# PaddlePaddle/PaddleRobotics

Measured on NVIDIA H100. Metric: env-steps/sec (A1, 4096 envs), higher is better.
Workload: dtype f32

## Files before the change

paddlerobotics_b200/csrc/b2q_api.cu:

```cuda
#include <cuda_runtime.h>
#include <cstdio>
#include <cstdlib>
#include <new>
#include <string>
#include "b2q_host_common.h"
#include "b2q_render_internal.h"
#include "../../include/b2q_render.h"

using namespace b2q;

namespace {

struct WarpComm {
  int k;
  unsigned char* scr;
  __device__ __forceinline__ int leg() const { return k; }
  template <typename T> __device__ __forceinline__ T* scratch() const { return reinterpret_cast<T*>(scr); }
  __device__ __forceinline__ void sync() const { __syncwarp(); }
  __device__ __forceinline__ bool any(bool f) const { return __any_sync(0xffffffffu, f) != 0; }
  template <typename T>
  __device__ __forceinline__ T sum4(T v) const {
    v += __shfl_xor_sync(0xffffffffu, v, 1);
    v += __shfl_xor_sync(0xffffffffu, v, 2);
    return v;
  }
  template <typename T>
  __device__ __forceinline__ T bcast(T v, int f) const { return __shfl_sync(0xffffffffu, v, f, 4); }
};

template <typename T>
__device__ __forceinline__ const Model<T>& stage_model(const Model<T>* g, unsigned char* smem) {
  Model<T>* s = reinterpret_cast<Model<T>*>(smem);
  const uint4* src = reinterpret_cast<const uint4*>(g);
  uint4* dst = reinterpret_cast<uint4*>(s);
  constexpr int NV = (int)((sizeof(Model<T>) + 15) / 16);
  for (int i0 = threadIdx.x; i0 < NV; i0 += 4 * blockDim.x) {
    uint4 v[4];
#pragma unroll
    for (int k = 0; k < 4; k++) { const int i = i0 + k * (int)blockDim.x; if (i < NV) v[k] = __ldg(src + i); }
#pragma unroll
    for (int k = 0; k < 4; k++) { const int i = i0 + k * (int)blockDim.x; if (i < NV) dst[i] = v[k]; }
  }
  __syncthreads();
  return *s;
}

template <typename T>
__device__ __forceinline__ void copy_block(T* __restrict__ dst, const T* stage, int n) {
  constexpr int PER = 16 / (int)sizeof(T);
  if ((((size_t)dst | (size_t)stage) & 15) == 0 && n % PER == 0) {
    uint4* d4 = reinterpret_cast<uint4*>(dst); const uint4* s4 = reinterpret_cast<const uint4*>(stage);
    for (int i = threadIdx.x; i < n / PER; i += blockDim.x) d4[i] = s4[i];
  } else {
    for (int i = threadIdx.x; i < n; i += blockDim.x) dst[i] = stage[i];
  }
}

template <typename T>
__device__ __forceinline__ void emit_obs_block(const Model<T>& md, const T* stage, T* __restrict__ obs, int env0, int rows) {
  const int od = md.obs_dim;
  T* dst = obs + (size_t)env0 * od;
  if (md.obs_identity) { copy_block(dst, stage, rows * OBS_DIM); return; }
  for (int i = threadIdx.x; i < rows * od; i += blockDim.x) { int r = i / od, j = i - r * od; dst[i] = obs_out_elem(md, stage + r * OBS_DIM, j); }
}

template <typename T, int FEAT>
__global__ void __launch_bounds__(128) b2q_step_kernel(Cfg<T> cf, const Model<T>* __restrict__ gm, Buffers<T> B, const T* __restrict__ action, int donef,
                                                       int auto_reset, T* __restrict__ obs, T* __restrict__ reward, uint8_t* __restrict__ done, T* __restrict__ info) {
  extern __shared__ __align__(32) unsigned char smem[];
  const Model<T>& md = stage_model(gm, smem);
  T* stage = reinterpret_cast<T*>(smem + ((sizeof(Model<T>) + 31) & ~size_t(31)));
  int gid = blockIdx.x * blockDim.x + threadIdx.x;
  int env = gid >> 2;
  const int env0 = (blockIdx.x * blockDim.x) >> 2, per_cta = blockDim.x >> 2;
  bool valid = env < B.N;
  const int srow = env0 + (int)(threadIdx.x >> 2);
  if (!valid) env = B.N - 1;
  T* istage0 = stage + (size_t)per_cta * OBS_DIM;
  WarpComm cm{(int)(threadIdx.x & 3), reinterpret_cast<unsigned char*>(istage0 + (size_t)per_cta * INFO_DIM + (size_t)(threadIdx.x >> 2) * scratch_floats(FEAT))};
  T* istage = istage0;
  step_lane<T, FEAT>(cm, cf, md, B, env, valid, action, donef, auto_reset, stage + (ptrdiff_t)(srow - env) * OBS_DIM, reward, done, istage, env0, env0);
  __syncthreads();
  const int rows = min(per_cta, B.N - env0);
  emit_obs_block(md, stage, obs, env0, rows);
  copy_block(info + (size_t)env0 * INFO_DIM, istage, rows * INFO_DIM);
}

template <typename T, int FEAT>
__global__ void __launch_bounds__(128) b2q_settle_kernel(Cfg<T> cf, const Model<T>* __restrict__ gm, Buffers<T> B, const uint8_t* __restrict__ mask) {
  extern __shared__ __align__(32) unsigned char smem[];
  const Model<T>& md = stage_model(gm, smem);
  int gid = blockIdx.x * blockDim.x + threadIdx.x;
  int env = gid >> 2;
  bool valid = env < B.N;
  if (!valid) env = B.N - 1;
  if (mask && !mask[env]) valid = false;
  T* scr0 = reinterpret_cast<T*>(smem + ((sizeof(Model<T>) + 31) & ~size_t(31))) + (size_t)(blockDim.x >> 2) * (OBS_DIM + INFO_DIM);
  WarpComm cm{(int)(threadIdx.x & 3), reinterpret_cast<unsigned char*>(scr0 + (size_t)(threadIdx.x >> 2) * scratch_floats(FEAT))};
  settle_lane<T, FEAT>(cm, cf, md, B, env, valid);
}

template <typename T>
__global__ void __launch_bounds__(128) b2q_reset_kernel(Cfg<T> cf, const Model<T>* __restrict__ gm, Buffers<T> B, const uint8_t* __restrict__ mask, const T* __restrict__ xoff,
                                                        T* __restrict__ obs) {
  extern __shared__ __align__(32) unsigned char smem[];
  const Model<T>& md = stage_model(gm, smem);
  T* stage = reinterpret_cast<T*>(smem + ((sizeof(Model<T>) + 31) & ~size_t(31)));
  int gid = blockIdx.x * blockDim.x + threadIdx.x;
  int env = gid >> 2;
  const int env0 = (blockIdx.x * blockDim.x) >> 2;
  bool valid = env < B.N;
  if (!valid) env = B.N - 1;
  if (mask && !mask[env]) valid = false;
  WarpComm cm{(int)(threadIdx.x & 3), nullptr};
  T* srow = stage + (size_t)(threadIdx.x >> 2) * OBS_DIM;
  reset_lane<T>(cm, cf, md, B, env, valid, obs ? srow : (T*)nullptr, xoff);
  if (obs) {
    __syncwarp();
    if (valid) { const int od = md.obs_dim; for (int j = threadIdx.x & 3; j < od; j += 4) obs[(size_t)env * od + j] = obs_out_elem(md, srow, j); }
  }
  (void)env0;
}

template <typename T>
__global__ void b2q_pack_param_kernel(const T* __restrict__ dyn, const T* __restrict__ def48, P4<T>* param, const uint8_t* __restrict__ mask, int N, T max_latency,
                                      int* __restrict__ overflow) {
  int env = blockIdx.x * blockDim.x + threadIdx.x;
  if (env >= N || (mask && !mask[env])) return;
  pack_param_env<T>(dyn, def48, param, N, env);
  const T lat = dyn ? dyn[(size_t)env * 48 + 25] : def48[25];
  if (!(lat <= max_latency)) atomicMax(overflow, 1);
}
template <typename T>
__global__ void b2q_pack_force_kernel(const T* __restrict__ f, P4<T>* extf, int N) {
// ... 46 lines not shown
  do {                                                                                \
    cudaError_t e_ = (call);                                                          \
    if (e_ != cudaSuccess) {                                                          \
      err = std::string(#call) + ": " + cudaGetErrorString(e_);                       \
      return B2Q_ECUDA;                                                               \
    }                                                                                 \
  } while (0)

template <typename T>
struct EnvT : EnvBase {
  Cfg<T> kc;
  Buffers<T> B;
  Model<T>* d_model = nullptr;
  T* d_def48 = nullptr;
  T* d_hf = nullptr;
  void* d_pool = nullptr;
  int tpb = 32;
  float hf_lo = 0.0f, hf_hi = 0.0f;

  ~EnvT() override {
    cudaSetDevice(cfg.device);
    if (d_pool) cudaFree(d_pool);
    if (d_model) cudaFree(d_model);
    if (d_def48) cudaFree(d_def48);
    if (d_hf) cudaFree(d_hf);
    if (st_act) cudaFree(st_act);
    if (h_flag) cudaFreeHost(h_flag);
  }
  int grid_lanes() const { return (B.N * 4 + tpb - 1) / tpb; }

  int init(const B2QConfig& c) {
    cfg = c; prec = c.precision;
    tpb = c.threads_per_block ? c.threads_per_block : 32;
    if (const char* e = std::getenv("B2Q_HOST_IO")) host_io = std::atoi(e);
    CK(cudaSetDevice(c.device));
    int N = c.num_envs, Dm = c.ring_depth;
    if (c.terrain_type == 1) {
      size_t n = (size_t)c.hf_nx * c.hf_ny;
      T* tmp = (T*)malloc(n * sizeof(T));
      if (!tmp) { err = "host alloc failed"; return B2Q_ENOMEM; }
      for (size_t i = 0; i < n; i++) tmp[i] = (T)c.hf_host[i];
      hf_lo = hf_hi = (float)tmp[0];
      for (size_t i = 0; i < n; i++) { hf_lo = std::fmin(hf_lo, (float)tmp[i]); hf_hi = std::fmax(hf_hi, (float)tmp[i]); }
      cudaError_t e1 = cudaMalloc(&d_hf, n * sizeof(T));
      if (e1 == cudaSuccess) e1 = cudaMemcpy(d_hf, tmp, n * sizeof(T), cudaMemcpyHostToDevice);
      free(tmp);
      CK(e1);
    }
    kc = make_cfg<T>(c, d_hf);
    Model<T> hm; build_model_host(hm, c.foot_radius, c.etg_T, c.etg_amp, c.etg_phase0, c.etg_phase1, c.etg_foot_y_inset);
    build_obs_map(hm, c); obs_dim = hm.obs_dim;
    feat = config_feat(c);
    if (feat) tpb = 32;
    if (smem_bytes() > 48 * 1024) {
      if (feat) {
        CK(cudaFuncSetAttribute(b2q_step_kernel<T, 1>, cudaFuncAttributeMaxDynamicSharedMemorySize, (int)smem_bytes()));
        CK(cudaFuncSetAttribute(b2q_settle_kernel<T, 1>, cudaFuncAttributeMaxDynamicSharedMemorySize, (int)smem_bytes()));
      } else {
        CK(cudaFuncSetAttribute(b2q_step_kernel<T, 0>, cudaFuncAttributeMaxDynamicSharedMemorySize, (int)smem_bytes()));
        CK(cudaFuncSetAttribute(b2q_settle_kernel<T, 0>, cudaFuncAttributeMaxDynamicSharedMemorySize, (int)smem_bytes()));
      }
    }
    CK(cudaHostAlloc((void**)&h_flag, sizeof(int), cudaHostAllocDefault));
    CK(cudaMalloc((void**)&d_model, (sizeof(Model<T>) + 15) / 16 * 16));
    CK(cudaMemset(d_model, 0, (sizeof(Model<T>) + 15) / 16 * 16));
    CK(cudaMemcpy(d_model, &hm, sizeof(Model<T>), cudaMemcpyHostToDevice));
    double d48[48]; default_dyn_row(d48); T t48[48]; for (int i = 0; i < 48; i++) t48[i] = (T)d48[i];
    CK(cudaMalloc(&d_def48, sizeof(t48)));
    CK(cudaMemcpy(d_def48, t48, sizeof(t48), cudaMemcpyHostToDevice));
    size_t packs = (size_t)(NS + NS + 12 + NP + NE + Dm * 24 + STUCK_H + 1) * N;
    size_t bytes = packs * sizeof(P4<T>) + (size_t)(N + 1) * sizeof(int);
    CK(cudaMalloc(&d_pool, bytes));
    CK(cudaMemset(d_pool, 0, bytes));
    P4<T>* p = (P4<T>*)d_pool;
    B.N = N; B.Dm = Dm;
    B.state = p; p += (size_t)NS * N; B.snap = p; p += (size_t)NS * N; B.snap_obs = p; p += (size_t)12 * N;
    B.param = p; p += (size_t)NP * N; B.etg = p; p += (size_t)NE * N; B.ring = p; p += (size_t)Dm * 24 * N;
    B.pos_hist = p; p += (size_t)STUCK_H * N; B.extf = p; p += (size_t)N;
    B.step_count = (int*)p; d_flag = B.step_count + N;
    int rc = set_dynamics(nullptr, nullptr, 0);
    if (rc) return rc;
    rc = reset(nullptr, nullptr, nullptr, nullptr, nullptr, 0);
    if (rc) return rc;
    CK(cudaDeviceSynchronize());
    return B2Q_OK;
  }
  size_t smem_bytes() const {
    return ((sizeof(Model<T>) + 31) & ~size_t(31)) + (size_t)(tpb / 4) * (OBS_DIM + INFO_DIM + scratch_floats(feat)) * sizeof(T);
  }

  int set_dynamics(const uint8_t* mask, const void* dyn, cudaStream_t s) override {
    CK(cudaSetDevice(cfg.device));
    int N = B.N;
    const double max_lat = ((double)B.Dm * cfg.action_repeat - 2) * cfg.sim_dt * (1.0 + 1e-9);
    CK(cudaMemsetAsync(d_flag, 0, sizeof(int), s));
    b2q_pack_param_kernel<T><<<(N + 127) / 128, 128, 0, s>>>((const T*)dyn, d_def48, const_cast<P4<T>*>(B.param), mask, N, (T)max_lat, d_flag);
    CK(cudaMemcpyAsync(h_flag, d_flag, sizeof(int), cudaMemcpyDeviceToHost, s));
    CK(cudaStreamSynchronize(s));
    launches += 1;
    if (*h_flag) {
      char buf[200];
      snprintf(buf, sizeof buf, "b2q_set_dynamics: a control_latency exceeds %.4f s, the most ring_depth=%d can serve (need ring_depth >= ceil((latency/sim_dt + 2) / action_repeat))", max_lat, B.Dm);
      err = buf;
      return B2Q_EINVAL;
    }
    if (feat) b2q_settle_kernel<T, 1><<<grid_lanes(), tpb, smem_bytes(), s>>>(kc, d_model, B, mask);
    else b2q_settle_kernel<T, 0><<<grid_lanes(), tpb, smem_bytes(), s>>>(kc, d_model, B, mask);
    launches += 1;
    CK(cudaGetLastError());
    return B2Q_OK;
  }
  int reset(const uint8_t* mask, const void* w, const void* b, const void* xoff, void* obs, cudaStream_t s) override {
    CK(cudaSetDevice(cfg.device));
    int N = B.N;
    if (w || b) { b2q_pack_etg_kernel<T><<<(N + 127) / 128, 128, 0, s>>>((const T*)w, (const T*)b, const_cast<P4<T>*>(B.etg), mask, N); launches++; }
    const size_t smem_reset = ((sizeof(Model<T>) + 31) & ~size_t(31)) + (size_t)(tpb / 4) * OBS_DIM * sizeof(T);
    b2q_reset_kernel<T><<<grid_lanes(), tpb, smem_reset, s>>>(kc, d_model, B, mask, (const T*)xoff, (T*)obs);
    launches++;
    CK(cudaGetLastError());
    return B2Q_OK;
  }
  int set_force(const void* f, cudaStream_t s) override {
    if (!cfg.external_force) { err = "b2q_set_external_force: the handle was created with external_force = 0"; return B2Q_EINVAL; }
    CK(cudaSetDevice(cfg.device));
    b2q_pack_force_kernel<T><<<(B.N + 127) / 128, 128, 0, s>>>((const T*)f, const_cast<P4<T>*>(B.extf), B.N);
    launches++;
    CK(cudaGetLastError());
    return B2Q_OK;
  }
  int feat = 0; int* d_flag = nullptr; int* h_flag = nullptr;
  int step(const void* action, int donef, void* obs, void* rew, uint8_t* done, void* info, cudaStream_t s) override {
    if (!action || !obs || !rew || !done || !info) { err = "b2q_step: null device pointer"; return B2Q_EINVAL; }
    { int cur = -1; if (cudaGetDevice(&cur) != cudaSuccess || cur != cfg.device) CK(cudaSetDevice(cfg.device)); }
    if (feat) b2q_step_kernel<T, 1><<<grid_lanes(), tpb, smem_bytes(), s>>>(kc, d_model, B, (const T*)action, donef, cfg.auto_reset, (T*)obs, (T*)rew, done, (T*)info);
    else b2q_step_kernel<T, 0><<<grid_lanes(), tpb, smem_bytes(), s>>>(kc, d_model, B, (const T*)action, donef, cfg.auto_reset, (T*)obs, (T*)rew, done, (T*)info);
    launches++;
    CK(cudaGetLastError());
    return B2Q_OK;
  }
  T* st_act = nullptr; T* st_obs = nullptr; T* st_rew = nullptr; uint8_t* st_done = nullptr; T* st_info = nullptr;
  int step_host(const void* a, int donef, void* obs, void* rew, uint8_t* done, void* info, cudaStream_t s) override {
    if (!a || !obs || !rew || !done) { err = "b2q_step_host: null host pointer"; return B2Q_EINVAL; }
    CK(cudaSetDevice(cfg.device));
    const size_t N = (size_t)B.N;
    if (!st_act) {
      size_t bytes = N * ((size_t)act_dim() + OBS_DIM + 1 + INFO_DIM) * sizeof(T) + N + 512;
      void* p = nullptr;
      CK(cudaMalloc(&p, bytes));
      st_act = (T*)p; st_obs = st_act + N * (size_t)act_dim(); st_rew = st_obs + N * OBS_DIM; st_done = (uint8_t*)(st_rew + N);
      st_info = (T*)((uint8_t*)p + ((N * ((size_t)act_dim() + OBS_DIM + 1) * sizeof(T) + N + 255) / 256) * 256);
    }
    const T* act_dev = st_act;
    if (host_io >= 1 && (act_dev = (const T*)mapped(a)) == nullptr) act_dev = st_act;
    if (act_dev == st_act) CK(cudaMemcpyAsync(st_act, a, N * (size_t)act_dim() * sizeof(T), cudaMemcpyHostToDevice, s));
    T* obs_dev = nullptr; T* rew_dev = nullptr; uint8_t* done_dev = nullptr;
    if (host_io >= 2) { obs_dev = (T*)mapped(obs); rew_dev = (T*)mapped(rew); done_dev = (uint8_t*)mapped(done); }
    const bool direct = obs_dev && rew_dev && done_dev;
    T* info_dev = (direct && info) ? (T*)mapped(info) : nullptr;
    int rc = direct ? step(act_dev, donef, obs_dev, rew_dev, done_dev, info_dev ? info_dev : st_info, s) : step(act_dev, donef, st_obs, st_rew, st_done, st_info, s);
    if (rc) return rc;
    if (info_dev) info = nullptr;
    const size_t b_obs = N * (size_t)obs_dim * sizeof(T), b_rew = N * sizeof(T);
    if (direct) {
    } else if ((uint8_t*)rew == (uint8_t*)obs + b_obs && done == (uint8_t*)rew + b_rew) {
      CK(cudaMemcpyAsync(obs, st_obs, b_obs + b_rew + N, cudaMemcpyDeviceToHost, s));
    } else {
      CK(cudaMemcpyAsync(obs, st_obs, b_obs, cudaMemcpyDeviceToHost, s));
      CK(cudaMemcpyAsync(rew, st_rew, b_rew, cudaMemcpyDeviceToHost, s));
      CK(cudaMemcpyAsync(done, st_done, N, cudaMemcpyDeviceToHost, s));
    }
    if (info) CK(cudaMemcpyAsync(info, st_info, N * INFO_DIM * sizeof(T), cudaMemcpyDeviceToHost, s));
    CK(cudaStreamSynchronize(s));
    return B2Q_OK;
  }
  int host_io = 2;
  void* mapped(const void* p) {
    cudaPointerAttributes at;
    if (cudaPointerGetAttributes(&at, p) == cudaSuccess && at.type == cudaMemoryTypeHost && at.devicePointer) return at.devicePointer;
    cudaGetLastError();
    return nullptr;
  }
  int get_state(void* out, cudaStream_t s) override {
    if (!out) { err = "b2q_get_state: null pointer"; return B2Q_EINVAL; }
    CK(cudaSetDevice(cfg.device));
    b2q_get_state_kernel<T><<<(B.N + 127) / 128, 128, 0, s>>>(B.state, (T*)out, B.N); launches++;
    CK(cudaGetLastError());
    return B2Q_OK;
// ... 98 lines not shown
```

paddlerobotics_b200/csrc/b2q_sim.cuh:

```cuda
#pragma once
#include "b2q_math.cuh"

namespace b2q {

constexpr int NS = 37;
constexpr int NP = 15;
constexpr int NE = 16;
constexpr int OBS_DIM = 49;
constexpr int INFO_DIM = 56;
constexpr int ETG_H = 20;

template <typename T>
struct alignas(4 * sizeof(T)) P4 {
  T x, y, z, w;
};

template <typename T>
struct LegModel {
  T p1[3];
  T lhip;
  T com[3][3];
  T I[3][6];
  T m[3];
};
template <typename T>
struct Model {
  LegModel<T> leg[4];
  T m0, I0[6];
  T foot_r, l_up, l_low;
  T etg_u[ETG_H][2];
  T base_foot[4][3];
  T etg_mean[12], etg_std[12], etg_istd[12];
  T pose_ori[3];
  T qlo[3], qhi[3];
  T knee_r;
  int obs_dim, obs_identity;
  int obs_src[OBS_DIM];
  T obs_scale[OBS_DIM], obs_shift[OBS_DIM];
};
template <typename T>
struct Cfg {
  T dt; int R; int iters; T erp, warm, margin; int interp; T tau_limit; int settle_steps;
  int filter; T fb0, fb1, fb2, fa1, fa2; int etg; int max_steps;
  T etg_T, etg_T2, etg_sigma_sq, etg_amp, etg_ph0, etg_ph1;
  T w_torso, w_feet, w_up, w_tau, w_stand, w_badfoot, w_footcontact, w_done, reward_p, vel_d;
  int terrain, hf_nx, hf_ny; T hf_x0, hf_y0, hf_cell, hf_icell, idt; const T* hf;
  int clip_cmd; T max_dq;
  int noise_on; T noise[5]; unsigned long long noise_seed;
  int stuck, body_coll;
  int motor_mode, jlim, extf, knee; T damp[4];
};
constexpr int STUCK_H = 10;
template <typename T>
struct Buffers {
  int N, Dm;
  P4<T>* state;
  P4<T>* snap;
  P4<T>* snap_obs;
  const P4<T>* param;
  const P4<T>* etg;
  P4<T>* ring;
  int* step_count;
  P4<T>* pos_hist;
  const P4<T>* extf;
};
template <typename T>
struct LaneParam {
// ... 44 lines not shown
  K.a2 = K.R1.cy;
  K.p1 = mk<T>(lm.p1[0], lm.p1[1], lm.p1[2]);
  K.p2 = K.p1 + K.R1.cy * lm.lhip;
  K.p3 = K.p2 - K.R2.cz * md.l_up;
  K.toe = K.p3 - K.R3m.cz * md.l_low;
}

template <typename T>
B2Q_HD void leg_ik(const Model<T>& md, V3<T> f, T lhip, T* ang) {
  T lu = md.l_up, ll = md.l_low;
  T tk = -m_acos((f.x * f.x + f.y * f.y + f.z * f.z - lhip * lhip - ll * ll - lu * lu) / (2 * ll * lu));
  T l = m_sqrt(lu * lu + ll * ll + 2 * lu * ll * m_cos(tk));
  T th = m_asin(-f.x / l) - tk / 2;
  T cc = m_cos(th + tk / 2);
  T c1 = lhip * f.y - l * cc * f.z;
  T s1 = l * cc * f.y + lhip * f.z;
  ang[0] = m_atan2(s1, c1); ang[1] = th; ang[2] = tk;
}

template <typename T, class Comm>
B2Q_HD void etg_act_leg(const Comm& cm, const Cfg<T>& cf, const Model<T>& md, const P4<T>* etg, int N, int env, T t, T* act) {
  const int k = cm.leg();
  if (!cf.etg) { act[0] = act[1] = act[2] = T(0); return; }
  const T two_pi = T(6.283185307179586476925286766559);
  T tt = (k == 0 || k == 3) ? t : t + T(0.5) * cf.etg_T2;
  T om = two_pi / cf.etg_T;
  T x0 = cf.etg_amp * m_sin(cf.etg_ph0 + om * tt), x1 = cf.etg_amp * m_sin(cf.etg_ph1 + om * tt);
  T d[3] = {0, 0, 0};
  const T isig = T(1) / cf.etg_sigma_sq;
  T e[4 * NE];
#pragma unroll
  for (int p = 0; p < NE; p++) { P4<T> v = ldp(etg, p, N, env); e[4 * p] = v.x; e[4 * p + 1] = v.y; e[4 * p + 2] = v.z; e[4 * p + 3] = v.w; }
#pragma unroll
  for (int h = 0; h < ETG_H; h++) {
    T dx = x0 - md.etg_u[h][0], dy = x1 - md.etg_u[h][1];
    T r = m_exp(-(dx * dx + dy * dy) * isig);
#pragma unroll
    for (int a = 0; a < 3; a++) d[a] += e[a * ETG_H + h] * r;
  }
#pragma unroll
  for (int a = 0; a < 3; a++) d[a] += e[60 + a];
  const LegModel<T>& lm = md.leg[k];
  T ang[3];
  for (int tries = 0; tries < 200; tries++) {
    V3<T> f = mk<T>(md.base_foot[k][0] + d[0] - lm.p1[0], md.base_foot[k][1] + d[1] - lm.p1[1], md.base_foot[k][2] + d[2] - lm.p1[2]);
    leg_ik(md, f, lm.lhip, ang);
    if (!(m_isnan(ang[0]) || m_isnan(ang[1]) || m_isnan(ang[2]))) break;
    d[0] *= T(0.95); d[1] *= T(0.95); d[2] *= T(0.95);
  }
#pragma unroll
  for (int a = 0; a < 3; a++) act[a] = ang[a] - md.pose_ori[a];
}

constexpr int RPL = 9, NRW = 4 * RPL;
constexpr int SCRATCH_FLOATS = NRW * 6 + 4 * 45 + NRW * 4 + NRW * NRW;
constexpr int SCRATCH_FAST = 272;
B2Q_HD constexpr int scratch_floats(int feat) { return feat ? SCRATCH_FLOATS : SCRATCH_FAST; }
#define JLIM_GAP T(0.06)
template <typename T, class Comm>
B2Q_HD void solve_rows36(const Comm& cm, const Cfg<T>& cf, T mu, const T (*Y)[6] , const T* u , const T* blk45 ,
                         const T* targ , const bool* act , const T* warm , T* lk ) {
  const int k = cm.leg();
  T* sh = cm.template scratch<T>();
  T* Ya = sh; T* blk = sh + NRW * 6; T* vec = blk + 4 * 45; T* W = vec + NRW * 4;
  cm.sync();
  for (int e = 0; e < RPL; e++) {
    const int r = RPL * k + e;
    for (int c = 0; c < 6; c++) Ya[r * 6 + c] = Y[e][c];
    vec[r * 4 + 0] = u[e]; vec[r * 4 + 1] = targ[e]; vec[r * 4 + 2] = act[e] ? T(1) : T(0); vec[r * 4 + 3] = warm[e];
  }
  for (int i = 0; i < 45; i++) blk[k * 45 + i] = blk45[i];
  cm.sync();
  const int grp_row[9] = {6, 7, 8, 0, 3, 1, 2, 4, 5}, grp_par[9] = {-1, -1, -1, -1, -1, 0, 0, 3, 3};
  int idx[NRW], par[NRW], pos_of[NRW], n = 0;
  for (int i = 0; i < NRW; i++) pos_of[i] = -1;
  for (int seg = 0; seg < 5; seg++) {
    const int g0 = seg == 0 ? 0 : seg == 1 ? 3 : seg == 2 ? 4 : seg == 3 ? 5 : 7, g1 = seg == 0 ? 3 : seg == 1 ? 4 : seg == 2 ? 5 : seg == 3 ? 7 : 9;
    for (int f = 0; f < 4; f++)
      for (int g = g0; g < g1; g++) {
        const int r = RPL * f + grp_row[g];
        if (!(vec[r * 4 + 2] > T(0))) continue;
        idx[n] = r; par[n] = grp_par[g] >= 0 ? pos_of[RPL * f + grp_par[g]] : -1; pos_of[r] = n; n++;
      }
  }
  for (int i = 0; i < n; i++) {
    const int r = idx[i];
    if (r / RPL != k) continue;
    for (int j = 0; j < n; j++) {
      const int c = idx[j];
      T acc = T(0);
      for (int q = 0; q < 6; q++) acc += Ya[r * 6 + q] * Ya[c * 6 + q];
      if (c / RPL == k) { const int a = r - RPL * k, b = c - RPL * k; acc += blk[k * 45 + (a >= b ? a * (a + 1) / 2 + b : b * (b + 1) / 2 + a)]; }
      W[i * NRW + j] = acc;
    }
  }
  cm.sync();
  T lam[NRW], uu[NRW];
  for (int i = 0; i < n; i++) lam[i] = vec[idx[i] * 4 + 3];
  for (int i = 0; i < n; i++) { T a = vec[idx[i] * 4 + 0]; for (int j = 0; j < n; j++) a += W[i * NRW + j] * lam[j]; uu[i] = a; }
  for (int it = 0; it < cf.iters; it++) {
    for (int i = 0; i < n; i++) {
      T ln = lam[i] + (vec[idx[i] * 4 + 1] - uu[i]) / W[i * NRW + i];
      if (par[i] >= 0) { T lim = mu * lam[par[i]]; ln = m_min(m_max(ln, -lim), lim); } else ln = m_max(ln, T(0));
      T dl = ln - lam[i]; lam[i] = ln;
      for (int j = 0; j < n; j++) uu[j] += W[j * NRW + i] * dl;
    }
  }
  for (int e = 0; e < RPL; e++) { const int q = pos_of[RPL * k + e]; lk[e] = q >= 0 ? lam[q] : T(0); }
  cm.sync();
}

template <typename T, int FEAT, class Comm>
B2Q_HD void substep(const Comm& cm, const Cfg<T>& cf, const Model<T>& md, const LaneParam<T>& pr, LaneState<T>& s,
                    const T* target, T* tau_out, V3<T> fext = V3<T>{0, 0, 0}, const T* hyb = nullptr ) {
  const int k = cm.leg();
  const LegModel<T>& lm = md.leg[k];
  const T dt = cf.dt, idt = cf.idt;
  R3<T> R = quat_to_R(s.qx, s.qy, s.qz, s.qw);
  V3<T> wB = rotT(R, s.vang), vB = rotT(R, s.vlin), gB = rotT(R, pr.g);

  T tau[3];
#pragma unroll
  for (int j = 0; j < 3; j++) {
    T cmd = target[j];
    if (cf.clip_cmd) cmd = m_min(m_max(cmd, s.q[j] - cf.max_dq), s.q[j] + cf.max_dq);
    T t = T(-1) * (pr.kp[j] * (s.q[j] - cmd)) - pr.kd[j] * (s.qd[j] - T(0));
    if (FEAT && cf.motor_mode == 1) t = target[j];
    if (FEAT && cf.motor_mode == 2) t = T(-1) * (hyb[j] * (s.q[j] - cmd)) - hyb[6 + j] * (s.qd[j] - hyb[3 + j]) + hyb[9 + j];
    if (cf.tau_limit > T(0)) t = m_min(m_max(t, -cf.tau_limit), cf.tau_limit);
    tau[j] = t; tau_out[j] = t;
  }

  LegKin<T> K; leg_kin(md, lm, s.q, K);
  const V3<T> a1 = mk<T>(1, 0, 0), a2 = K.a2;
  V3<T> cL[3]; S3<T> IL[3]; T mL[3];
  {
    const R3<T>* Rs[3] = {&K.R1, &K.R2, &K.R3m};
    const V3<T> ps[3] = {K.p1, K.p2, K.p3};
#pragma unroll
    for (int i = 0; i < 3; i++) {
      cL[i] = ps[i] + rot(*Rs[i], mk<T>(lm.com[i][0], lm.com[i][1], lm.com[i][2]));
      S3<T> Il = {lm.I[i][0], lm.I[i][1], lm.I[i][2], lm.I[i][3], lm.I[i][4], lm.I[i][5]};
      S3<T> Ib = rot_sym(*Rs[i], Il);
      T sc = pr.iscale[i];
      IL[i].xx = Ib.xx * sc; IL[i].xy = Ib.xy * sc; IL[i].xz = Ib.xz * sc; IL[i].yy = Ib.yy * sc; IL[i].yz = Ib.yz * sc; IL[i].zz = Ib.zz * sc;
      mL[i] = lm.m[i] * pr.mscale[i];
    }
  }
  V3<T> w1 = wB + a1 * s.qd[0], w2 = w1 + a2 * s.qd[1], w3 = w2 + a2 * s.qd[2];
  V3<T> pdd0 = cross(wB, vB) - gB;
  V3<T> al1 = cross(wB, a1) * s.qd[0];
  V3<T> pdd1 = pdd0 + cross(wB, cross(wB, K.p1));
  V3<T> al2 = al1 + cross(w1, a2) * s.qd[1];
  V3<T> d21 = K.p2 - K.p1;
  V3<T> pdd2 = pdd1 + cross(al1, d21) + cross(w1, cross(w1, d21));
  V3<T> al3 = al2 + cross(w2, a2) * s.qd[2];
  V3<T> d32 = K.p3 - K.p2;
  V3<T> pdd3 = pdd2 + cross(al2, d32) + cross(w2, cross(w2, d32));
  V3<T> fL[3], nL[3];
  {
    const V3<T> ws[3] = {w1, w2, w3}, als[3] = {al1, al2, al3}, pdds[3] = {pdd1, pdd2, pdd3}, ps[3] = {K.p1, K.p2, K.p3};
#pragma unroll
    for (int i = 0; i < 3; i++) {
      V3<T> r = cL[i] - ps[i];
      V3<T> cdd = pdds[i] + cross(als[i], r) + cross(ws[i], cross(ws[i], r));
      fL[i] = cdd * mL[i];
      nL[i] = mul(IL[i], als[i]) + cross(ws[i], mul(IL[i], ws[i]));
// ... 168 lines not shown
        V3<T> xk = K.p3 - ek[0] * md.knee_r;
        V3<T> r1 = cross(a1, xk - K.p1), r2 = cross(a2, xk - K.p2), r3 = cross(a2, xk - K.p3);
#pragma unroll
        for (int e = 0; e < 3; e++) {
          T jr[3] = {dot(ek[e], r1), dot(ek[e], r2), dot(ek[e], r3)};
          V6<T> Jb; Jb.a = cross(xk, ek[e]); Jb.l = ek[e];
          u9[3 + e] = dot(Jb.a, wBs) + dot(Jb.l, vBs) + jr[0] * qds[0] + jr[1] * qds[1] + jr[2] * qds[2];
#pragma unroll
          for (int i = 0; i < 6; i++) Yx[e][i] = get6(Jb, i) - (FD[0][i] * jr[0] + FD[1][i] * jr[1] + FD[2][i] * jr[2]);
          fwd6(S, Li, Yx[e]);
          Jx[e][0] = jr[0]; Jx[e][1] = jr[1]; Jx[e][2] = jr[2];
          targ9[3 + e] = T(0); warm9[3 + e] = T(0); act9[3 + e] = kact;
        }
        targ9[3] = kdist > T(0) ? -kdist * idt : cf.erp * (-kdist) * idt;
      }
#pragma unroll
      for (int j = 0; j < 3; j++) {
        T glo = s.q[j] - md.qlo[j], ghi = md.qhi[j] - s.q[j], gap = glo, sj = T(1);
        if (ghi < glo) { gap = ghi; sj = T(-1); }
#pragma unroll
        for (int i = 0; i < 6; i++) Yx[3 + j][i] = -sj * FD[j][i];
        fwd6(S, Li, Yx[3 + j]);
        Jx[3 + j][0] = j == 0 ? sj : T(0); Jx[3 + j][1] = j == 1 ? sj : T(0); Jx[3 + j][2] = j == 2 ? sj : T(0);
        u9[6 + j] = sj * qds[j];
        targ9[6 + j] = gap > T(0) ? -gap * idt : cf.erp * (-gap) * idt;
        warm9[6 + j] = cf.warm * s.lam_lim[j];
        act9[6 + j] = cf.jlim && (gap < JLIM_GAP);
      }
#pragma unroll
      for (int e = 0; e < 6; e++) {
#pragma unroll
        for (int c = 0; c < 6; c++) Y9[3 + e][c] = Yx[e][c];
        Jall[3 + e][0] = Jx[e][0]; Jall[3 + e][1] = Jx[e][1]; Jall[3 + e][2] = Jx[e][2];
      }
#pragma unroll
      for (int a = 0; a < RPL; a++) {
        T dj[3];
#pragma unroll
        for (int i = 0; i < 3; i++) dj[i] = D[i][0] * Jall[a][0] + D[i][1] * Jall[a][1] + D[i][2] * Jall[a][2];
#pragma unroll
        for (int b = 0; b <= a; b++) blk[a * (a + 1) / 2 + b] = Jall[b][0] * dj[0] + Jall[b][1] * dj[1] + Jall[b][2] * dj[2];
      }
      T lk9[RPL];
      solve_rows36<T>(cm, cf, pr.mu, Y9, u9, blk, targ9, act9, warm9, lk9);
#pragma unroll
      for (int e = 0; e < 3; e++) lk[e] = lk9[e];
#pragma unroll
      for (int e = 0; e < 6; e++) lkx[e] = lk9[3 + e];
      general = true;
    }
  }
  if (!general) {
  T g[12], Wc[12][12], lam[12];
  {
    T* sh = cm.template scratch<T>();
    T* YT = sh;
    T* vecs = sh + 72;
    T* afs = sh + 120;
    T* Wp = sh + 128;
    const T targ_n = dist > T(0) ? -dist * idt : cf.erp * (-dist) * idt;
    T invo[3];
#pragma unroll
    for (int e = 0; e < 3; e++) {
      T d = Wl[e][e];
#pragma unroll
      for (int c = 0; c < 6; c++) d = m_fma(Y[e][c], Y[e][c], d);
      invo[e] = act ? m_rcp(d) : T(0);
      const int i = 3 * k + e;
#pragma unroll
      for (int c = 0; c < 6; c++) YT[c * 12 + i] = Y[e][c];
      vecs[i] = invo[e]; vecs[12 + i] = u[e]; vecs[24 + i] = e == 0 ? targ_n : T(0);
      vecs[36 + i] = (e == 0 && act) ? cf.warm * s.lam_n : T(0);
    }
    afs[k] = act ? T(1) : T(0);
    cm.sync();
    {
      T Ya[12][6], inv[12];
#pragma unroll
      for (int c = 0; c < 6; c++) {
#pragma unroll
        for (int q = 0; q < 3; q++) {
          const P4<T> v = *reinterpret_cast<const P4<T>*>(YT + c * 12 + 4 * q);
          Ya[4 * q][c] = v.x; Ya[4 * q + 1][c] = v.y; Ya[4 * q + 2][c] = v.z; Ya[4 * q + 3][c] = v.w;
        }
      }
#pragma unroll
      for (int q = 0; q < 3; q++) { const P4<T> v = *reinterpret_cast<const P4<T>*>(vecs + 4 * q); inv[4 * q] = v.x; inv[4 * q + 1] = v.y; inv[4 * q + 2] = v.z; inv[4 * q + 3] = v.w; }
#pragma unroll
      for (int e = 0; e < 3; e++) {
        const int r = 3 * k + e;
        T col[12];
#pragma unroll
        for (int i = 0; i < 12; i++) {
          T acc = Ya[i][0] * Y[e][0];
#pragma unroll
          for (int c = 1; c < 6; c++) acc = m_fma(Ya[i][c], Y[e][c], acc);
          col[i] = acc * inv[i];
        }
#pragma unroll
        for (int q = 0; q < 3; q++) { P4<T> v; v.x = col[4 * q]; v.y = col[4 * q + 1]; v.z = col[4 * q + 2]; v.w = col[4 * q + 3]; *reinterpret_cast<P4<T>*>(Wp + r * 12 + 4 * q) = v; }
#pragma unroll
        for (int e2 = 0; e2 < 3; e2++) {
          T w = Wl[e2][e];
#pragma unroll
          for (int c = 0; c < 6; c++) w = m_fma(Y[e2][c], Y[e][c], w);
          Wp[r * 12 + 3 * k + e2] = (e2 == e) ? T(0) : w * invo[e2];
        }
      }
    }
    cm.sync();
#pragma unroll
    for (int r = 0; r < 12; r++) {
#pragma unroll
      for (int q = 0; q < 3; q++) { const P4<T> v = *reinterpret_cast<const P4<T>*>(Wp + r * 12 + 4 * q); Wc[r][4 * q] = v.x; Wc[r][4 * q + 1] = v.y; Wc[r][4 * q + 2] = v.z; Wc[r][4 * q + 3] = v.w; }
    }
    {
      const P4<T> af = *reinterpret_cast<const P4<T>*>(afs);
      const T actf[4] = {af.x, af.y, af.z, af.w};
      T lw[4];
#pragma unroll
      for (int q = 0; q < 3; q++) {
        const P4<T> iv = *reinterpret_cast<const P4<T>*>(vecs + 4 * q), uv = *reinterpret_cast<const P4<T>*>(vecs + 12 + 4 * q);
        const P4<T> tv = *reinterpret_cast<const P4<T>*>(vecs + 24 + 4 * q), lv = *reinterpret_cast<const P4<T>*>(vecs + 36 + 4 * q);
        g[4 * q] = (tv.x - uv.x) * iv.x; g[4 * q + 1] = (tv.y - uv.y) * iv.y; g[4 * q + 2] = (tv.z - uv.z) * iv.z; g[4 * q + 3] = (tv.w - uv.w) * iv.w;
        lam[4 * q] = lv.x; lam[4 * q + 1] = lv.y; lam[4 * q + 2] = lv.z; lam[4 * q + 3] = lv.w;
      }
#pragma unroll
      for (int f = 0; f < 4; f++) lw[f] = lam[3 * f];
#pragma unroll
      for (int i = 0; i < 12; i++) {
#pragma unroll
        for (int f = 0; f < 4; f++) g[i] = m_fma(Wc[3 * f][i], -lw[f], g[i]);
        if (i % 3 == 0 && !(actf[i / 3] > T(0))) g[i] = T(-1e30);
      }
    }
    cm.sync();
  }
  for (int it = 0; it < cf.iters; it++) {
#pragma unroll
    for (int f = 0; f < 4; f++) {
      const int r = 3 * f;
      T ln = m_max(g[r], T(0));
      T dl = lam[r] - ln; lam[r] = ln;
#pragma unroll
      for (int i = 0; i < 12; i++)
        if (i != r) g[i] = m_fma(Wc[r][i], dl, g[i]);
    }
#pragma unroll
    for (int f = 0; f < 4; f++) {
#pragma unroll
      for (int td = 1; td < 3; td++) {
        const int r = 3 * f + td;
        T lim = pr.mu * lam[3 * f];
        T ln = m_min(m_max(g[r], -lim), lim);
        T dl = lam[r] - ln; lam[r] = ln;
#pragma unroll
        for (int i = 0; i < 12; i++)
          if (i != r) g[i] = m_fma(Wc[r][i], dl, g[i]);
      }
    }
  }
#pragma unroll
  for (int f = 0; f < 4; f++) if (f == k) { lk[0] = lam[3 * f]; lk[1] = lam[3 * f + 1]; lk[2] = lam[3 * f + 2]; }
  }
  s.lam_n = lk[0]; s.contact = lk[0] > T(0); s.lam_lim[0] = lkx[3]; s.lam_lim[1] = lkx[4]; s.lam_lim[2] = lkx[5];
  T z[6];
#pragma unroll
  for (int c = 0; c < 6; c++) z[c] = cm.sum4(Y[0][c] * lk[0] + Y[1][c] * lk[1] + Y[2][c] * lk[2] + (FEAT != 0 ? Yx[0][c] * lkx[0] + Yx[1][c] * lkx[1] + Yx[2][c] * lkx[2] + Yx[3][c] * lkx[3] + Yx[4][c] * lkx[4] + Yx[5][c] * lkx[5] : T(0)));
  bwd6(S, Li, z);
  V6<T> dnu = arr_to_v6(z);
  {
    T jl[3], t[3];
#pragma unroll
    for (int i = 0; i < 3; i++) {
      jl[i] = Jk[0][i] * lk[0] + Jk[1][i] * lk[1] + Jk[2][i] * lk[2];
      if (FEAT != 0) jl[i] += Jx[0][i] * lkx[0] + Jx[1][i] * lkx[1] + Jx[2][i] * lkx[2] + Jx[3][i] * lkx[3] + Jx[4][i] * lkx[4] + Jx[5][i] * lkx[5];
      t[i] = jl[i] - dot6(Fc[i], dnu);
    }
#pragma unroll
    for (int j = 0; j < 3; j++) qds[j] += D[j][0] * t[0] + D[j][1] * t[1] + D[j][2] * t[2];
  }
  wBs = wBs + dnu.a; vBs = vBs + dnu.l;
  s.vang = rot(R, wBs); s.vlin = rot(R, vBs);
#pragma unroll
  for (int j = 0; j < 3; j++) { s.qd[j] = qds[j]; s.q[j] += dt * qds[j]; }
  s.pos = s.pos + s.vlin * dt;
  {
    T wx = s.vang.x, wy = s.vang.y, wz = s.vang.z, th = m_sqrt(wx * wx + wy * wy + wz * wz) * dt;
    T sh, cw; sincos_t(T(0.5) * th, sh, cw);
    T kk = th < T(1e-4) ? T(0.5) - th * th * T(1.0 / 48.0) : sh * m_rcp(th);
    T dx = wx * dt * kk, dy = wy * dt * kk, dz = wz * dt * kk;
    T ox = cw * s.qx + dx * s.qw + dy * s.qz - dz * s.qy;
    T oy = cw * s.qy - dx * s.qz + dy * s.qw + dz * s.qx;
    T oz = cw * s.qz + dx * s.qy - dy * s.qx + dz * s.qw;
    T ow = cw * s.qw - dx * s.qx - dy * s.qy - dz * s.qz;
    T nn = m_rsqrt(ox * ox + oy * oy + oz * oz + ow * ow);
    s.qx = ox * nn; s.qy = oy * nn; s.qz = oz * nn; s.qw = ow * nn;
  }
}

template <typename T> B2Q_HD P4<T> ldp(const P4<T>* base, int pack, int N, int env) { return base[(size_t)pack * N + env]; }
template <typename T> B2Q_HD void stp(P4<T>* base, int pack, int N, int env, T x, T y, T z, T w) {
  P4<T> p; p.x = x; p.y = y; p.z = z; p.w = w; base[(size_t)pack * N + env] = p;
}

template <typename T, class Comm>
B2Q_HD void load_param(const Comm& cm, const Buffers<T>& B, int env, LaneParam<T>& pr) {
  const int k = cm.leg(), N = B.N;
  P4<T> a = ldp(B.param, 0 + k, N, env), b = ldp(B.param, 4 + k, N, env), c = ldp(B.param, 8 + k, N, env);
  P4<T> d = ldp(B.param, 12, N, env), e = ldp(B.param, 13, N, env), g = ldp(B.param, 14, N, env);
  pr.kp[0] = a.x; pr.kp[1] = a.y; pr.kp[2] = a.z; pr.mu = a.w;
  pr.kd[0] = b.x; pr.kd[1] = b.y; pr.kd[2] = b.z; pr.latency = b.w;
  pr.iscale[0] = c.x; pr.iscale[1] = c.y; pr.iscale[2] = c.z;
  pr.mscale[0] = d.x; pr.mscale[1] = d.y; pr.mscale[2] = d.z; pr.m0s = d.w;
  pr.I0s[0] = e.x; pr.I0s[1] = e.y; pr.I0s[2] = e.z;
  pr.g = mk<T>(g.x, g.y, g.z);
// ... 72 lines not shown

template <typename T> B2Q_HD T obs_out_elem(const Model<T>& md, const T* full49, int j) {
  return md.obs_identity ? full49[j] : full49[md.obs_src[j]] * md.obs_scale[j] + md.obs_shift[j];
}

template <typename T, class Comm>
B2Q_HD void reset_lane(const Comm& cm, const Cfg<T>& cf, const Model<T>& md, const Buffers<T>& B, int env, bool valid, T* obs ,
                       const T* xoff = nullptr ) {
  const int k = cm.leg(), N = B.N;
  LaneState<T> s; T la[3], ea[3]; int hl; V3<T> rpy0;
  load_state(cm, B.snap, N, env, s, la, ea, hl, rpy0);
  T sq[3], sqd[3], stau[3];
  {
    P4<T> a = ldp(B.snap_obs, 3 * k, N, env), b = ldp(B.snap_obs, 3 * k + 1, N, env), c = ldp(B.snap_obs, 3 * k + 2, N, env);
    sq[0] = a.x; sq[1] = a.y; sq[2] = a.z; stau[0] = a.w; sqd[0] = b.x; sqd[1] = b.y; sqd[2] = b.z; stau[1] = b.w; stau[2] = c.x;
  }
  s.contact = s.lam_n > T(0);
  if (xoff) s.pos.x += xoff[env];
  rpy0 = quat_to_rpy(s.qx, s.qy, s.qz, s.qw);
  etg_act_leg(cm, cf, md, B.etg, N, env, T(0), ea);
  la[0] = la[1] = la[2] = T(0);
  if (valid) {
    store_state(cm, B.state, N, env, s, la, ea, 0, rpy0);
    for (int d = 0; d < B.Dm; d++) { ring_write(B, d, 0, k, env, sq, sqd, stau); ring_write(B, d, 1, k, env, sq, sqd, stau); }
    if (k == 0) B.step_count[env] = 0;
    if (cf.filter) for (int hslot = 0; hslot < 4; hslot++) stp(B.state, 21 + 4 * k + hslot, N, env, sq[0], sq[1], sq[2], T(0));
  }
  if (obs) write_obs(cm, md, obs, valid, s, s.pos, cf.dt * T(cf.R), rpy0, sq, sqd, ea);
}

template <typename T, int FEAT, class Comm>
B2Q_HD void settle_lane(const Comm& cm, const Cfg<T>& cf, const Model<T>& md, const Buffers<T>& B, int env, bool valid) {
  const int k = cm.leg(), N = B.N;
  LaneParam<T> pr; load_param(cm, B, env, pr);
  LaneState<T> s;
  s.pos = mk<T>(0, 0, T(0.32)); s.qx = s.qy = s.qz = 0; s.qw = 1; s.vlin = mk<T>(0, 0, 0); s.vang = mk<T>(0, 0, 0);
  T tgt[3], tau[3] = {0, 0, 0};
#pragma unroll
  for (int j = 0; j < 3; j++) { s.q[j] = md.pose_ori[j]; s.qd[j] = 0; tgt[j] = md.pose_ori[j]; }
  s.lam_n = 0; s.contact = 0; s.lam_lim[0] = s.lam_lim[1] = s.lam_lim[2] = 0;
  Cfg<T> cs = cf; cs.motor_mode = 0;
#pragma unroll 1
  for (int i = 0; i < cf.settle_steps; i++) substep<T, FEAT>(cm, cs, md, pr, s, tgt, tau);
  s.lam_lim[0] = s.lam_lim[1] = s.lam_lim[2] = T(0);
  if (valid) {
    T z3[3] = {0, 0, 0};
    store_state(cm, B.snap, N, env, s, z3, z3, 0, mk<T>(0, 0, 0));
    stp(B.snap_obs, 3 * k + 0, N, env, s.q[0], s.q[1], s.q[2], tau[0]);
    stp(B.snap_obs, 3 * k + 1, N, env, s.qd[0], s.qd[1], s.qd[2], tau[1]);
    stp(B.snap_obs, 3 * k + 2, N, env, tau[2], T(0), T(0), T(0));
  }
}

template <typename T, int FEAT, class Comm>
B2Q_HD void step_lane(const Comm& cm, const Cfg<T>& cf, const Model<T>& md, const Buffers<T>& B, int env, bool valid,
                      const T* action, int donef, int auto_reset, T* obs, T* reward, uint8_t* done, T* info, int obs_env0 = 0, int info_env0 = 0) {
  const int k = cm.leg(), N = B.N, R = cf.R;
  const T dtc = cf.dt * T(R);
  LaneParam<T> pr; load_param(cm, B, env, pr);
  LaneState<T> s; T last_action[3], etg_act[3]; int has_last; V3<T> rpy0;
  load_state(cm, B.state, N, env, s, last_action, etg_act, has_last, rpy0);
  int step = B.step_count[env];
  T target[3];
#pragma unroll
  for (int j = 0; j < 3; j++) target[j] = md.pose_ori[j] + etg_act[j] + action[(size_t)env * 12 + 3 * k + j];
  V3<T> fext = mk<T>(0, 0, 0);
  if (FEAT) {
    if (cf.motor_mode == 1) {
#pragma unroll
      for (int j = 0; j < 3; j++) target[j] = action[(size_t)env * 12 + 3 * k + j];
    }
    if (cf.extf) { P4<T> f = B.extf[env]; fext = mk<T>(f.x, f.y, f.z); }
  }
  T hyb[12] = {0, 0, 0, 0, 0, 0, 0, 0, 0, 0, 0, 0};
  if (FEAT && cf.motor_mode == 2) {
#pragma unroll
    for (int j = 0; j < 3; j++) {
      const T* a5 = action + ((size_t)env * 12 + 3 * k + j) * 5;
      target[j] = a5[0]; hyb[j] = a5[1]; hyb[3 + j] = a5[2]; hyb[6 + j] = a5[3]; hyb[9 + j] = a5[4];
    }
  }
  if (cf.filter && !(FEAT && cf.motor_mode == 2)) {
    P4<T> x1 = ldp(B.state, 21 + 4 * k, N, env), x2 = ldp(B.state, 22 + 4 * k, N, env), y1 = ldp(B.state, 23 + 4 * k, N, env), y2 = ldp(B.state, 24 + 4 * k, N, env);
    T ax1[3] = {x1.x, x1.y, x1.z}, ax2[3] = {x2.x, x2.y, x2.z}, ay1[3] = {y1.x, y1.y, y1.z}, ay2[3] = {y2.x, y2.y, y2.z}, yy[3];
#pragma unroll
    for (int j = 0; j < 3; j++) yy[j] = cf.fb0 * target[j] + cf.fb1 * ax1[j] + cf.fb2 * ax2[j] - cf.fa1 * ay1[j] - cf.fa2 * ay2[j];
    if (valid) {
      stp(B.state, 21 + 4 * k, N, env, target[0], target[1], target[2], T(0)); stp(B.state, 22 + 4 * k, N, env, ax1[0], ax1[1], ax1[2], T(0));
      stp(B.state, 23 + 4 * k, N, env, yy[0], yy[1], yy[2], T(0)); stp(B.state, 24 + 4 * k, N, env, ay1[0], ay1[1], ay1[2], T(0));
    }
#pragma unroll
    for (int j = 0; j < 3; j++) target[j] = yy[j];
  }
  const V3<T> start_pos = s.pos;
  T foot0_x;
  {
    LegKin<T> K; leg_kin(md, md.leg[k], s.q, K);
    R3<T> Rb = quat_to_R(s.qx, s.qy, s.qz, s.qw);
    foot0_x = s.pos.x + rot(Rb, K.toe).x;
  }
  int n_lag = pr.latency > T(0) ? (int)(pr.latency / cf.dt) : 0;
  T alpha = pr.latency > T(0) ? (pr.latency - T(n_lag) * cf.dt) / cf.dt : T(0);
  int max_lag = B.Dm * R - 2; if (n_lag > max_lag) { n_lag = max_lag; alpha = T(0); }
  int ia = ((R - 1 - n_lag) % R + R) % R, ma = (n_lag - (R - 1 - ia)) / R;
  int ib = ((R - 2 - n_lag) % R + R) % R, mb = (n_lag + 1 - (R - 1 - ib)) / R;
  const int slot = step % B.Dm;
  T tau[3] = {0, 0, 0};
#pragma unroll 1
  for (int i = 0; i < R; i++) {
    T proc[3];
    if (cf.interp && has_last && !(FEAT && cf.motor_mode == 2)) {
      T lerp = T(i + 1) / T(R);
#pragma unroll
      for (int j = 0; j < 3; j++) proc[j] = last_action[j] + lerp * (target[j] - last_action[j]);
    } else {
#pragma unroll
      for (int j = 0; j < 3; j++) proc[j] = target[j];
    }
    substep<T, FEAT>(cm, cf, md, pr, s, proc, tau, fext, hyb);
    if (valid && i == ia) ring_write(B, slot, 0, k, env, s.q, s.qd, tau);
    if (valid && i == ib) ring_write(B, slot, 1, k, env, s.q, s.qd, tau);
  }
#pragma unroll
  for (int j = 0; j < 3; j++) last_action[j] = target[j];
  has_last = 1;
  T dq[3], dqd[3], dtau[3];
  {
    T aq[3], aqd[3], at[3], bq[3], bqd[3], bt[3];
    ring_read(B, ((step - ma) % B.Dm + B.Dm) % B.Dm, 0, k, env, aq, aqd, at);
    ring_read(B, ((step - mb) % B.Dm + B.Dm) % B.Dm, 1, k, env, bq, bqd, bt);
#pragma unroll
    for (int j = 0; j < 3; j++) {
      dq[j] = (T(1) - alpha) * aq[j] + alpha * bq[j];
      dqd[j] = (T(1) - alpha) * aqd[j] + alpha * bqd[j];
      dtau[j] = (T(1) - alpha) * at[j] + alpha * bt[j];
    }
  }
  step += 1;
  T nz6[6] = {0, 0, 0, 0, 0, 0};
  if (cf.noise_on) {
    T n4[4];
    philox_normal4<T>(cf.noise_seed, (uint32_t)env, (uint32_t)step, (uint32_t)(16 * k + 0), n4);
#pragma unroll
    for (int j = 0; j < 3; j++) dq[j] += cf.noise[0] * n4[j];
    philox_normal4<T>(cf.noise_seed, (uint32_t)env, (uint32_t)step, (uint32_t)(16 * k + 1), n4);
#pragma unroll
    for (int j = 0; j < 3; j++) dqd[j] += cf.noise[1] * n4[j];
    philox_normal4<T>(cf.noise_seed, (uint32_t)env, (uint32_t)step, (uint32_t)(16 * k + 2), n4);
#pragma unroll
    for (int j = 0; j < 3; j++) dtau[j] += cf.noise[2] * n4[j];
    if (k == 0) {
      philox_normal4<T>(cf.noise_seed, (uint32_t)env, (uint32_t)step, 64u, n4);
      nz6[0] = cf.noise[3] * n4[0]; nz6[1] = cf.noise[3] * n4[1]; nz6[2] = cf.noise[3] * n4[2];
      philox_normal4<T>(cf.noise_seed, (uint32_t)env, (uint32_t)step, 65u, n4);
      nz6[3] = cf.noise[4] * n4[0]; nz6[4] = cf.noise[4] * n4[1]; nz6[5] = cf.noise[4] * n4[2];
    }
  }
  etg_act_leg(cm, cf, md, B.etg, N, env, T(step) * dtc, etg_act);
  T* orow = obs + (size_t)(env - obs_env0) * OBS_DIM;
  write_obs(cm, md, orow, valid, s, start_pos, dtc, rpy0, dq, dqd, etg_act, cf.noise_on ? nz6 : (const T*)nullptr);

  R3<T> Rb = quat_to_R(s.qx, s.qy, s.qz, s.qw);
  LegKin<T> K; leg_kin(md, md.leg[k], s.q, K);
  V3<T> toe_w = s.pos + rot(Rb, K.toe), knee_w = s.pos + rot(Rb, K.p3), nrm;
  const T idtc = T(1) / dtc;
  T velx = (s.pos.x - start_pos.x) * idtc;
  T torso = m_min(velx, cf.vel_d);
  T feet = cm.sum4(m_min((toe_w.x - foot0_x) * idtc, cf.vel_d) * T(0.25));
  V3<T> rpy = quat_to_rpy(s.qx, s.qy, s.qz, s.qw);
  T up = T(1) - T(0.5) * (c_prec(rpy.x, T(0), T(0.25)) + c_prec(rpy.y, T(0), T(0.25)));
  T pw = cm.sum4(dtau[0] * dqd[0] + dtau[1] * dqd[1] + dtau[2] * dqd[2]);
  T energy = m_abs(pw) * cf.dt * T(R);
// ... 68 lines not shown
```

Baseline: 33.74 million.

## Add split PGS sweep that keeps only normal rows and own tangents per lane

Adds a SPLIT variant of the contact solve. The Delassus matrix is written in a permuted layout: four normal columns, then two tangent columns per foot. Each lane then keeps only the normal rows and its own two tangent columns instead of the full 12x12 W and 12 impulses, with tangent updates broadcast across the four leg lanes. It is meant to cut registers and FLOPs in the PGS loop, and is enabled only for the default feature path when the grid is large relative to the SM count. In exchange it adds shuffle broadcasts per foot per iteration and changes the sweep order slightly.

```diff
diff --git a/paddlerobotics_b200/csrc/b2q_api.cu b/paddlerobotics_b200/csrc/b2q_api.cu
--- a/paddlerobotics_b200/csrc/b2q_api.cu
+++ b/paddlerobotics_b200/csrc/b2q_api.cu
@@ -64,7 +64,7 @@
   for (int i = threadIdx.x; i < rows * od; i += blockDim.x) { int r = i / od, j = i - r * od; dst[i] = obs_out_elem(md, stage + r * OBS_DIM, j); }
 }
 
-template <typename T, int FEAT>
+template <typename T, int FEAT, bool SPLIT = false>
 __global__ void __launch_bounds__(128) b2q_step_kernel(Cfg<T> cf, const Model<T>* __restrict__ gm, Buffers<T> B, const T* __restrict__ action, int donef,
                                                        int auto_reset, T* __restrict__ obs, T* __restrict__ reward, uint8_t* __restrict__ done, T* __restrict__ info) {
   extern __shared__ __align__(32) unsigned char smem[];
@@ -79,7 +79,7 @@
   T* istage0 = stage + (size_t)per_cta * OBS_DIM;
   WarpComm cm{(int)(threadIdx.x & 3), reinterpret_cast<unsigned char*>(istage0 + (size_t)per_cta * INFO_DIM + (size_t)(threadIdx.x >> 2) * scratch_floats(FEAT))};
   T* istage = istage0;
-  step_lane<T, FEAT>(cm, cf, md, B, env, valid, action, donef, auto_reset, stage + (ptrdiff_t)(srow - env) * OBS_DIM, reward, done, istage, env0, env0);
+  step_lane<T, FEAT, SPLIT>(cm, cf, md, B, env, valid, action, donef, auto_reset, stage + (ptrdiff_t)(srow - env) * OBS_DIM, reward, done, istage, env0, env0);
   __syncthreads();
   const int rows = min(per_cta, B.N - env0);
   emit_obs_block(md, stage, obs, env0, rows);
@@ -232,12 +232,16 @@
     build_obs_map(hm, c); obs_dim = hm.obs_dim;
     feat = config_feat(c);
     if (feat) tpb = 32;
+    int sms = 0;
+    CK(cudaDeviceGetAttribute(&sms, cudaDevAttrMultiProcessorCount, c.device));
+    split = !feat && (long long)((N * 4 + tpb - 1) / tpb) * (tpb / 32) > 4LL * sms;
     if (smem_bytes() > 48 * 1024) {
       if (feat) {
         CK(cudaFuncSetAttribute(b2q_step_kernel<T, 1>, cudaFuncAttributeMaxDynamicSharedMemorySize, (int)smem_bytes()));
         CK(cudaFuncSetAttribute(b2q_settle_kernel<T, 1>, cudaFuncAttributeMaxDynamicSharedMemorySize, (int)smem_bytes()));
       } else {
         CK(cudaFuncSetAttribute(b2q_step_kernel<T, 0>, cudaFuncAttributeMaxDynamicSharedMemorySize, (int)smem_bytes()));
+        CK(cudaFuncSetAttribute(b2q_step_kernel<T, 0, true>, cudaFuncAttributeMaxDynamicSharedMemorySize, (int)smem_bytes()));
         CK(cudaFuncSetAttribute(b2q_settle_kernel<T, 0>, cudaFuncAttributeMaxDynamicSharedMemorySize, (int)smem_bytes()));
       }
     }
@@ -308,11 +312,12 @@
     CK(cudaGetLastError());
     return B2Q_OK;
   }
-  int feat = 0; int* d_flag = nullptr; int* h_flag = nullptr;
+  int feat = 0, split = 0; int* d_flag = nullptr; int* h_flag = nullptr;
   int step(const void* action, int donef, void* obs, void* rew, uint8_t* done, void* info, cudaStream_t s) override {
     if (!action || !obs || !rew || !done || !info) { err = "b2q_step: null device pointer"; return B2Q_EINVAL; }
     { int cur = -1; if (cudaGetDevice(&cur) != cudaSuccess || cur != cfg.device) CK(cudaSetDevice(cfg.device)); }
     if (feat) b2q_step_kernel<T, 1><<<grid_lanes(), tpb, smem_bytes(), s>>>(kc, d_model, B, (const T*)action, donef, cfg.auto_reset, (T*)obs, (T*)rew, done, (T*)info);
+    else if (split) b2q_step_kernel<T, 0, true><<<grid_lanes(), tpb, smem_bytes(), s>>>(kc, d_model, B, (const T*)action, donef, cfg.auto_reset, (T*)obs, (T*)rew, done, (T*)info);
     else b2q_step_kernel<T, 0><<<grid_lanes(), tpb, smem_bytes(), s>>>(kc, d_model, B, (const T*)action, donef, cfg.auto_reset, (T*)obs, (T*)rew, done, (T*)info);
     launches++;
     CK(cudaGetLastError());
diff --git a/paddlerobotics_b200/csrc/b2q_sim.cuh b/paddlerobotics_b200/csrc/b2q_sim.cuh
--- a/paddlerobotics_b200/csrc/b2q_sim.cuh
+++ b/paddlerobotics_b200/csrc/b2q_sim.cuh
@@ -13,6 +13,10 @@
 template <typename T>
 struct alignas(4 * sizeof(T)) P4 {
   T x, y, z, w;
+};
+template <typename T>
+struct alignas(2 * sizeof(T)) P2 {
+  T x, y;
 };
 
 template <typename T>
@@ -163,6 +167,43 @@
   for (int a = 0; a < 3; a++) act[a] = ang[a] - md.pose_ori[a];
 }
 
+template <typename T, class Comm>
+B2Q_HD void pgs_sweep_feet(const Comm& cm, int iters, T mu, const T (&Wn)[12][4], const T (&Wt)[12][2], T (&gn)[4], T (&gt)[2], T (&ln)[4], T (&lt)[2]) {
+  const int k = cm.leg();
+  for (int it = 0; it < iters; it++) {
+#pragma unroll
+    for (int f = 0; f < 4; f++) {
+      const int r = 3 * f;
+      const T c = m_max(gn[f], T(0));
+      const T dl = ln[f] - c; ln[f] = c;
+#pragma unroll
+      for (int j = 0; j < 4; j++)
+        if (j != f) gn[j] = m_fma(Wn[r][j], dl, gn[j]);
+      gt[0] = m_fma(Wt[r][0], dl, gt[0]); gt[1] = m_fma(Wt[r][1], dl, gt[1]);
+    }
+#pragma unroll
+    for (int f = 0; f < 4; f++) {
+      const int r1 = 3 * f + 1, r2 = 3 * f + 2;
+      const bool own = k == f;
+      const T lim = mu * ln[f];
+      const T c1 = m_min(m_max(gt[0], -lim), lim);
+      const T d1 = lt[0] - c1;
+      const T c2 = m_min(m_max(m_fma(Wt[r1][1], d1, gt[1]), -lim), lim);
+      const T d2 = lt[1] - c2;
+      if (own) { lt[0] = c1; lt[1] = c2; }
+      const T dl1 = cm.bcast(d1, f), dl2 = cm.bcast(d2, f);
+#pragma unroll
+      for (int j = 0; j < 4; j++) gn[j] = m_fma(Wn[r1][j], dl1, gn[j]);
+      if (!own) gt[0] = m_fma(Wt[r1][0], dl1, gt[0]);
+      gt[1] = m_fma(Wt[r1][1], dl1, gt[1]);
+#pragma unroll
+      for (int j = 0; j < 4; j++) gn[j] = m_fma(Wn[r2][j], dl2, gn[j]);
+      gt[0] = m_fma(Wt[r2][0], dl2, gt[0]);
+      if (!own) gt[1] = m_fma(Wt[r2][1], dl2, gt[1]);
+    }
+  }
+}
+
 constexpr int RPL = 9, NRW = 4 * RPL;
 constexpr int SCRATCH_FLOATS = NRW * 6 + 4 * 45 + NRW * 4 + NRW * NRW;
 constexpr int SCRATCH_FAST = 272;
@@ -221,9 +262,10 @@
   cm.sync();
 }
 
-template <typename T, int FEAT, class Comm>
+template <typename T, int FEAT, bool SPLIT = false, class Comm>
 B2Q_HD void substep(const Comm& cm, const Cfg<T>& cf, const Model<T>& md, const LaneParam<T>& pr, LaneState<T>& s,
                     const T* target, T* tau_out, V3<T> fext = V3<T>{0, 0, 0}, const T* hyb = nullptr ) {
+  static_assert(!SPLIT || FEAT == 0, "the split sweep is a variant of the default body");
   const int k = cm.leg();
   const LegModel<T>& lm = md.leg[k];
   const T dt = cf.dt, idt = cf.idt;
@@ -498,6 +540,7 @@
   }
   if (!general) {
   T g[12], Wc[12][12], lam[12];
+  T gn[4], gt[2], lamn[4], lamt[2], Wn[12][4], Wt[12][2];
   {
     T* sh = cm.template scratch<T>();
     T* YT = sh;
@@ -543,18 +586,50 @@
           for (int c = 1; c < 6; c++) acc = m_fma(Ya[i][c], Y[e][c], acc);
           col[i] = acc * inv[i];
         }
+        if constexpr (SPLIT) {
+          P4<T> v;
+          v.x = col[0]; v.y = col[3]; v.z = col[6]; v.w = col[9]; *reinterpret_cast<P4<T>*>(Wp + r * 12) = v;
+          v.x = col[1]; v.y = col[2]; v.z = col[4]; v.w = col[5]; *reinterpret_cast<P4<T>*>(Wp + r * 12 + 4) = v;
+          v.x = col[7]; v.y = col[8]; v.z = col[10]; v.w = col[11]; *reinterpret_cast<P4<T>*>(Wp + r * 12 + 8) = v;
+        } else {
 #pragma unroll
         for (int q = 0; q < 3; q++) { P4<T> v; v.x = col[4 * q]; v.y = col[4 * q + 1]; v.z = col[4 * q + 2]; v.w = col[4 * q + 3]; *reinterpret_cast<P4<T>*>(Wp + r * 12 + 4 * q) = v; }
+        }
 #pragma unroll
         for (int e2 = 0; e2 < 3; e2++) {
           T w = Wl[e2][e];
 #pragma unroll
           for (int c = 0; c < 6; c++) w = m_fma(Y[e2][c], Y[e][c], w);
-          Wp[r * 12 + 3 * k + e2] = (e2 == e) ? T(0) : w * invo[e2];
+          Wp[r * 12 + (SPLIT ? (e2 == 0 ? k : 4 + 2 * k + e2 - 1) : 3 * k + e2)] = (e2 == e) ? T(0) : w * invo[e2];
         }
       }
     }
     cm.sync();
+    if constexpr (SPLIT) {
+#pragma unroll
+      for (int r = 0; r < 12; r++) {
+        const P4<T> v = *reinterpret_cast<const P4<T>*>(Wp + r * 12);
+        const P2<T> t = *reinterpret_cast<const P2<T>*>(Wp + r * 12 + 4 + 2 * k);
+        Wn[r][0] = v.x; Wn[r][1] = v.y; Wn[r][2] = v.z; Wn[r][3] = v.w; Wt[r][0] = t.x; Wt[r][1] = t.y;
+      }
+      const P4<T> af = *reinterpret_cast<const P4<T>*>(afs);
+      const T actf[4] = {af.x, af.y, af.z, af.w};
+#pragma unroll
+      for (int f = 0; f < 4; f++) { const int i = 3 * f; gn[f] = (vecs[24 + i] - vecs[12 + i]) * vecs[i]; lamn[f] = vecs[36 + i]; }
+#pragma unroll
+      for (int e = 0; e < 2; e++) { const int i = 3 * k + 1 + e; gt[e] = (vecs[24 + i] - vecs[12 + i]) * vecs[i]; lamt[e] = vecs[36 + i]; }
+#pragma unroll
+      for (int j = 0; j < 4; j++) {
+#pragma unroll
+        for (int f = 0; f < 4; f++) gn[j] = m_fma(Wn[3 * f][j], -lamn[f], gn[j]);
+        if (!(actf[j] > T(0))) gn[j] = T(-1e30);
+      }
+#pragma unroll
+      for (int e = 0; e < 2; e++) {
+#pragma unroll
+        for (int f = 0; f < 4; f++) gt[e] = m_fma(Wt[3 * f][e], -lamn[f], gt[e]);
+      }
+    } else {
 #pragma unroll
     for (int r = 0; r < 12; r++) {
 #pragma unroll
@@ -580,8 +655,15 @@
         if (i % 3 == 0 && !(actf[i / 3] > T(0))) g[i] = T(-1e30);
       }
     }
+    }
     cm.sync();
   }
+  if constexpr (SPLIT) {
+  pgs_sweep_feet<T>(cm, cf.iters, pr.mu, Wn, Wt, gn, gt, lamn, lamt);
+  lk[1] = lamt[0]; lk[2] = lamt[1];
+#pragma unroll
+  for (int f = 0; f < 4; f++) if (f == k) lk[0] = lamn[f];
+  } else {
   for (int it = 0; it < cf.iters; it++) {
 #pragma unroll
     for (int f = 0; f < 4; f++) {
@@ -608,6 +690,7 @@
   }
 #pragma unroll
   for (int f = 0; f < 4; f++) if (f == k) { lk[0] = lam[3 * f]; lk[1] = lam[3 * f + 1]; lk[2] = lam[3 * f + 2]; }
+  }
   }
   s.lam_n = lk[0]; s.contact = lk[0] > T(0); s.lam_lim[0] = lkx[3]; s.lam_lim[1] = lkx[4]; s.lam_lim[2] = lkx[5];
   T z[6];
@@ -786,7 +869,7 @@
   }
 }
 
-template <typename T, int FEAT, class Comm>
+template <typename T, int FEAT, bool SPLIT = false, class Comm>
 B2Q_HD void step_lane(const Comm& cm, const Cfg<T>& cf, const Model<T>& md, const Buffers<T>& B, int env, bool valid,
                       const T* action, int donef, int auto_reset, T* obs, T* reward, uint8_t* done, T* info, int obs_env0 = 0, int info_env0 = 0) {
   const int k = cm.leg(), N = B.N, R = cf.R;
@@ -851,7 +934,7 @@
 #pragma unroll
       for (int j = 0; j < 3; j++) proc[j] = target[j];
     }
-    substep<T, FEAT>(cm, cf, md, pr, s, proc, tau, fext, hyb);
+    substep<T, FEAT, SPLIT>(cm, cf, md, pr, s, proc, tau, fext, hyb);
     if (valid && i == ia) ring_write(B, slot, 0, k, env, s.q, s.qd, tau);
     if (valid && i == ib) ring_write(B, slot, 1, k, env, s.q, s.qd, tau);
   }
```

After: 33.30 million, median of 6. Within noise of the previous version (-1.3%).
